# aleksandrina-streltsova/lidar-global-registration

Hardware: AMD Instinct MI355X
Metric: scan-pair registrations/sec (higher is better)
Workload: dtype f32

## Files before the change

lidar-global-registration_amd/csrc/lgr_match.hip:

```cpp
#include <rocprim/device/device_radix_sort.hpp>
#include <rocprim/device/device_scan.hpp>

#include <algorithm>
#include <vector>

#include "lgr_internal.h"

#include "lgr_match_common.cuh"
#include "lgr_match_cluster.cuh"
#include "lgr_match_pack.cuh"
#include "lgr_match_mfma.cuh"
#include "lgr_match_sweep.cuh"
#include "lgr_match_bounds.cuh"
#include "lgr_match_rerank.cuh"

extern "C" int lgr_match_last_stats(lgr_ctx* ctx, unsigned* out6) {
    if (!ctx || !out6) return LGR_ERR_INVALID_ARG;
    const lgr_match_stats& s = ctx->mstats;
    out6[0] = s.items_ab; out6[1] = s.dense_ab; out6[2] = s.items_ba;
    out6[3] = s.dense_ba; out6[4] = (unsigned) s.sub_cols; out6[5] = (unsigned) s.rg_rows;
    return LGR_OK;
}
extern "C" int lgr_match_last_work(lgr_ctx* ctx, double* executed_fraction) {
    if (!ctx || !executed_fraction) return LGR_ERR_INVALID_ARG;
// ... 347 lines not shown
    MaskStats* scratch_stats() const { return (MaskStats*) lb_part; }
};

struct CheckView {
    const uint8_t *done = nullptr, *sched = nullptr;
    const float* lb = nullptr;
    const unsigned* ustage = nullptr;
    const float *uq_rows = nullptr, *uq_cols = nullptr;
};

static const float betas[] = {LGR_PRUNE_BETAS};
static const int n_beta = (int) (sizeof betas / sizeof betas[0]);
static_assert(sizeof betas / sizeof betas[0] == 1, "LGR_PRUNE_BETAS: one final pass only (lgr_match_common.cuh)");
static_assert(sizeof betas / sizeof betas[0] + 1 <= 7, "MaskStats: slot 7 holds the stages counted once");

struct MatchCall {
    lgr_ctx* const ctx;
    const float* const d_a; const int ma;
    const float* const d_b; const int mb;
    const int block;
    int32_t* const d_ab_idx; float* const d_ab_dist; int32_t* const d_ba_idx; float* const d_ba_dist;
    const bool both;
    const lgr_match_options& mo;
    lgr_match_stats& st;
    const int near_t;
    const bool prune;
    MatchPrep* const P;
    const Side& A;
    Side B;
    int sub = 1, n_leaves = 0, rg_rows = BLOCK_ROWS;
    float *cen = nullptr, *cen2 = nullptr;
    char* misc = nullptr;
    int ma_pad = 0, mb_pad = 0, ta = 0, tb = 0, n_rb = 0, n_stage_total = 0, n_cc = 0, n_rg = 0, n_groups = 0, n_cpad = 0;
    float *sortedA = nullptr, *sortedB = nullptr;
    bool boxes = false;
    float *boxA = nullptr, *boxBt = nullptr;
    unsigned* rmax2 = nullptr;
    Fork aux;
    bool f16 = false, force_dense = false;
    OperandScale os{};
    int KS = 0, NF = 0;
    size_t bset_stride = 0, cset_stride = 0;
    char *Aop = nullptr, *Bop = nullptr;
    float *nAp = nullptr, *nBp = nullptr;
    float2 *shellA = nullptr, *shellB = nullptr;
    unsigned* d_max = nullptr;
    float *gmaxB = nullptr, *gmaxA = nullptr;
    int *cl_of_rg = nullptr, *tile_group = nullptr, *tile_leaf = nullptr, *group_start = nullptr;
    int *group_leaf = nullptr, *leaf_g0 = nullptr;
    Fork sB;
    PruneWs W{};
    int *rowmin = nullptr, *colmin = nullptr;
    unsigned long long *bestA = nullptr, *bestB = nullptr;
    int item_rb = 0, n_ir = 0, ccx = 0, n_flags = 0, mfma_grid = 0;
    int *iflags = nullptr, *ipos = nullptr;
    int2* ilist = nullptr;
    int *xcd_start = nullptr, *xcd_ctr = nullptr;
    unsigned kept_cap = 0;
    uint2* kept = nullptr;
    unsigned long long* kept_count = nullptr;
    unsigned short* ucol16 = nullptr;
    bool split_used = false;
    bool colstage = false, coarse = false;
    CoarseArgs ca_on{};
    ShellArgs shell{}, shell0{};
    const uint8_t* sched_final = nullptr;
    const unsigned long long* cur_pass_stages = nullptr;
    bool defer_init = false;
    CompView comp_rows{nullptr, 0, nullptr}, comp_cols{nullptr, 0, nullptr};
    CheckView chk;

    MatchCall(lgr_ctx* ctx, const float* d_a, int ma, const float* d_b, int mb, int block, int32_t* d_ab_idx, float* d_ab_dist, int32_t* d_ba_idx, float* d_ba_dist)
        : ctx(ctx), d_a(d_a), ma(ma), d_b(d_b), mb(mb), block(block), d_ab_idx(d_ab_idx), d_ab_dist(d_ab_dist), d_ba_idx(d_ba_idx), d_ba_dist(d_ba_dist),
          both(d_ba_idx != nullptr && mb > 0), mo(ctx->mopt), st(ctx->mstats), near_t(mo.near > 0 ? mo.near : NEAR_T),
          prune(mo.prune == 1 || (mo.prune != 0 && (double) ma * mb >= 65536.0 * 65536.0)),
          P(match_prep_of(ctx)), A(P->A) {}

    int build_both(const IrrRef* irr);
    int build_sides();
    int start_aux();
    int launch_sorted_copies(bool behind_main);
    int join_sorted();
    int choose_format();
    int upload_group_tables();
    PruneWs carve_prune_ws(char* base) const;
    int prepare_prune_ws();
    int pack_operands();
    int alloc_tables();
    int launch_mfma(const unsigned* mask, const CoarseArgs& ca, bool allow_split = true);
    int init_touched_tables();
    int run_dense();
    int lower_bounds();
    int coarse_setup();
    int near_schedule();
    CoarseArgs with_bounds() const;
    void build_comp();
    int upper_bounds_schedule(int pass);
    int init_pass_tables(int pass);
    int build_masks(int pass);
    int run_pruned();
    int read_back_stats();
    int irregular_rows();
    int self_check(const CheckView& v);
    int rerank();
};

#include "lgr_match_debug.cuh"

int MatchCall::build_both(const IrrRef* irr) {
    return lgr_run_pair(ctx, [&](lgr_ctx* cx) { return build_side(cx, d_a, ma, P->cen, P->cen2, P->sub, 1, P->rg_rows, WS_MATCH_NA, WS_MATCH_AP, 0, irr, &P->A); },
                        [&](lgr_ctx* cx) { return build_side(cx, d_b, mb, P->cen, P->cen2, P->sub, TILE, PAD, WS_MATCH_NB, WS_MATCH_BP, 1, irr, &B); });
}
int MatchCall::build_sides() {
    const bool prepared = P->armed && P->d_a == d_a && P->ma == ma && P->mb == mb && P->both == both && memcmp(&P->mopt, &mo, sizeof mo) == 0;
    P->armed = false;
    if (!prepared) LGR_TRY(match_cluster(ctx, d_a, ma, d_b, mb, both, true, P));
    LGR_TRY(build_both(P->irr));
    if (A.n_irr > IRR_CAP || B.n_irr > IRR_CAP || ((A.n_irr || B.n_irr) && (A.n_valid == 0 || B.n_valid == 0))) {
        st.irr_gave_up = 1u;
        LGR_TRY(build_both(nullptr));
    }
    st.irr_a = (unsigned) A.n_irr; st.irr_b = (unsigned) B.n_irr;
    sub = P->sub; n_leaves = KCL * sub; rg_rows = P->rg_rows;
    cen = P->cen; cen2 = P->cen2;
    LGR_TRY(lgr_ws_t(ctx, WS_MATCH_MISC, 8192, &misc));
    if (A.n_valid == 0 || B.n_valid == 0) return LGR_OK;
    ma_pad = A.n_pad; mb_pad = B.n_pad;
    st.rg_rows = rg_rows;
    ta = ma_pad / TILE; tb = mb_pad / TILE;
    n_rb = ma_pad / BLOCK_ROWS; n_stage_total = mb_pad / STAGE_COLS;
    return LGR_OK;
}

int MatchCall::start_aux() {
    LGR_TRY(lgr_ws_t(ctx, WS_MATCH_SORTED_B, (size_t) mb_pad * 33, &sortedB));
    if (both || prune) LGR_TRY(lgr_ws_t(ctx, WS_MATCH_SORTED_A, (size_t) ma_pad * 33, &sortedA));
    boxes = prune && mo.box_bounds != 0;
    if (boxes) {
        LGR_TRY(lgr_ws_t(ctx, WS_MATCH_BOX, (size_t) n_rb * 66 + (size_t) n_leaves * 66 + 64, &boxA));
        boxBt = boxA + (size_t) n_rb * 66;
        rmax2 = (unsigned*) (boxBt + (size_t) n_leaves * 66);
    }
    LGR_TRY(lgr_ctx_aux(ctx));
    aux.start(ctx, ctx->aux->stream, ctx->aux_ev, true);
    LGR_TRY(aux.fork(ctx->aux_ev));
    if (boxes) {
        const float* basis = P->basis;
        LGR_HIP(ctx, hipMemsetAsync(rmax2, 0, 4, aux.s));
        box_kernel<<<n_rb, 256, 0, aux.s>>>(d_a, A.perm, nullptr, n_rb, basis, basis + 33 * 33, 0, boxA, rmax2);
        box_kernel<<<n_leaves, 256, 0, aux.s>>>(d_b, B.perm, B.leaf_start, n_leaves, basis, basis + 33 * 33, 1, boxBt, rmax2);
        LGR_HIP(ctx, hipEventRecord(ctx->ev[30], aux.s));
    }
    LGR_HIP(ctx, hipGetLastError());
    return LGR_OK;
}
int MatchCall::launch_sorted_copies(bool behind_main) {
    if (aux.recorded) return LGR_OK;
    if (behind_main) LGR_TRY(aux.fork(ctx->ev[26]));
    gather_rows_kernel<<<cdiv((long long) mb_pad * 33, 256), 256, 0, aux.s>>>(d_b, B.perm, mb_pad, sortedB);
    if (sortedA) gather_rows_kernel<<<cdiv((long long) ma_pad * 33, 256), 256, 0, aux.s>>>(d_a, A.perm, ma_pad, sortedA);
    LGR_HIP(ctx, hipGetLastError());
    return aux.record();
}
int MatchCall::join_sorted() {
    LGR_TRY(launch_sorted_copies(false));
    return aux.join();
}

int MatchCall::choose_format() {
    f16 = mo.operand_format != 0;
    LGR_TRY(lgr_ws_t(ctx, WS_MATCH_NORMS, (size_t) ma_pad + (size_t) KCL * mb_pad + 2 * ((size_t) ta + (size_t) KCL * tb) + 64, &nAp));
    nBp = nAp + ma_pad;
    shellA = (float2*) (nBp + (size_t) KCL * mb_pad);
    shellB = shellA + ta;
    d_max = (unsigned*) (misc + 128);
    LGR_HIP(ctx, hipMemsetAsync(d_max, 0, 12, ctx->stream));
    const float r2 = std::max(A.nstat_n2, B.nstat_n2), drop2 = std::max(A.nstat_drop, B.nstat_drop);
    if (f16) force_dense = A.nstat_ovf || B.nstat_ovf;
    os = operand_scale(f16, r2, drop2, mo.operand_format);
    if (f16 && env_int("LGR_MATCH_DEBUG", 0))
        fprintf(stderr, "[lgr] operand statistics: max |x - c|^2 %.6g, dropped energy %.6g (A %.6g, B %.6g) -> %s; irregular rows %d + %d\n", (double) r2, (double) drop2,
                (double) A.nstat_drop, (double) B.nstat_drop, os.rot ? "rotated" : "plain", A.n_irr, B.n_irr);
    st.f16 = f16 ? (os.rot ? 2 : 1) : 0;
    KS = !f16 ? OpFmt<FMT_F32>::KS : os.rot ? OpFmt<FMT_F16R>::KS : OpFmt<FMT_F16>::KS;
    NF = !f16 ? OpFmt<FMT_F32>::NF : os.rot ? OpFmt<FMT_F16R>::NF : OpFmt<FMT_F16>::NF;
    const size_t frag_bytes = f16 ? sizeof(f16x8) : sizeof(float);
    const size_t a_op_bytes = (size_t) ta * NF * 64 * frag_bytes;
    bset_stride = (size_t) tb * NF * 64;
    LGR_TRY(lgr_ws_t(ctx, WS_MATCH_ROWMIN, a_op_bytes + 256, &Aop));
    const size_t b_op_bytes = KCL * bset_stride * frag_bytes;
    LGR_TRY(lgr_ws_t(ctx, WS_MATCH_COLMIN, b_op_bytes + 256, &Bop));
    n_rg = cdiv(ma_pad, rg_rows);
    return LGR_OK;
}

int MatchCall::upload_group_tables() {
    std::vector<int> h_group_start, h_tiles(2 * (size_t) tb);
    int group_cols = GROUP_COLS;
    while (group_cols < 65536 && ((size_t) mb_pad / group_cols + n_leaves) * (size_t) ma_pad * 4 > ((size_t) 24 << 30)) group_cols *= 2;
    for (int l = 0; l < n_leaves; ++l)
        for (int s0 = B.h_leaf_start[l]; s0 < B.h_leaf_start[l + 1]; s0 += group_cols) {
            int s1 = std::min(B.h_leaf_start[l + 1], s0 + group_cols), g = (int) h_group_start.size();
            h_group_start.push_back(s0);
            for (int t = s0 / TILE; t < s1 / TILE; ++t) { h_tiles[t] = g; h_tiles[tb + t] = l; }
        }
    n_groups = (int) h_group_start.size();
    st.sub_cols = n_groups;
    h_group_start.push_back(mb_pad);
    LGR_TRY(lgr_ws_t(ctx, WS_MATCH_BEST_B, (size_t) KCL * n_groups + 2 * (size_t) n_rg + 2 * (size_t) tb + 2 * (size_t) n_groups + n_leaves + 72, &gmaxB));
    gmaxA = gmaxB + (size_t) KCL * n_groups;
    cl_of_rg = (int*) (gmaxA + n_rg);
    tile_group = cl_of_rg + n_rg;
    tile_leaf = tile_group + tb;
    group_start = tile_leaf + tb;
    group_leaf = group_start + n_groups + 1;
    leaf_g0 = group_leaf + n_groups;
    std::vector<int> h(n_rg), hgl(n_groups), hl(n_leaves + 1, n_groups);
    for (int g = 0; g < n_rg; ++g) h[g] = A.h_blkcl[(size_t) g * (rg_rows / BLOCK_ROWS)];
    for (int g = 0; g < n_groups; ++g) hgl[g] = h_tiles[tb + h_group_start[g] / TILE];
    for (int g = n_groups - 1; g >= 0; --g) hl[hgl[g]] = g;
    for (int l = n_leaves - 1; l >= 0; --l) hl[l] = std::min(hl[l], hl[l + 1]);
    LGR_HIP(ctx, hipMemcpyAsync(cl_of_rg, h.data(), h.size() * 4, hipMemcpyHostToDevice, ctx->stream));
    LGR_HIP(ctx, hipMemcpyAsync(tile_group, h_tiles.data(), h_tiles.size() * 4, hipMemcpyHostToDevice, ctx->stream));
    LGR_HIP(ctx, hipMemcpyAsync(group_start, h_group_start.data(), h_group_start.size() * 4, hipMemcpyHostToDevice, ctx->stream));
    LGR_HIP(ctx, hipMemcpyAsync(group_leaf, hgl.data(), hgl.size() * 4, hipMemcpyHostToDevice, ctx->stream));
    LGR_HIP(ctx, hipMemcpyAsync(leaf_g0, hl.data(), hl.size() * 4, hipMemcpyHostToDevice, ctx->stream));
    LGR_HIP(ctx, hipStreamSynchronize(ctx->stream));
    return LGR_OK;
}

static void launch_pack16(bool rot, hipStream_t s, const float* X, const int* perm, int n_pad, int role, const float* cen, const int* blkcl, const F16Scale& sc,
                          void* op, float* nrm, float2* shell) {
    if (rot) pack16_kernel<true><<<cdiv(n_pad, 256), 256, 0, s>>>(X, perm, n_pad, role, cen, blkcl, sc, (_Float16*) op, nrm, shell);
    else pack16_kernel<false><<<cdiv(n_pad, 256), 256, 0, s>>>(X, perm, n_pad, role, cen, blkcl, sc, (_Float16*) op, nrm, shell);
}

PruneWs MatchCall::carve_prune_ws(char* base) const {
    Carve carve{0, base};
    PruneWs w{};
    const size_t n_pairs = (size_t) n_rb * n_leaves;
    w.LBsq = carve.take<float>(n_pairs * 4);
    w.done = carve.take<uint8_t>(n_pairs);
    w.sched = carve.take<uint8_t>(n_pairs);
    w.touched = carve.take<uint8_t>(n_pairs);
    w.mask = carve.take<unsigned>((size_t) n_rb * n_cc * 4);
    w.mask_acc = carve.take<unsigned>((size_t) n_rb * n_cc * 4);
    w.u_rb = carve.take<float>((size_t) n_rb * 4);
    w.u_rt = carve.take<float>((size_t) n_rb * (BLOCK_ROWS / TILE) * 4);
    w.u_leaf = carve.take<unsigned>((size_t) MAXLEAF * 4);
    w.stats = carve.take<MaskStats>(sizeof(MaskStats));
    w.lb_part = carve.take<uint2>((size_t) n_rb * sizeof(uint2));
    w.leaf_first = carve.take<int>((size_t) MAXLEAF * 4);
    w.leaf_last = carve.take<int>((size_t) MAXLEAF * 4);
    w.mask_chk = carve.take<unsigned>(mo.self_check ? (size_t) 2 * n_rb * n_cc * 4 + 256 : 0);
    w.u_stage = carve.take<unsigned>((size_t) n_stage_total * 4);
    w.u_ct = carve.take<unsigned>((size_t) tb * 4);
    w.comp_r = carve.take<uint8_t>((size_t) n_rb * n_groups);
    w.comp_c = carve.take<uint8_t>((size_t) n_leaves * n_rg);
    w.smaxB = carve.take<float>((size_t) KCL * n_stage_total * 4);
    w.coarse_cnt = carve.take<unsigned long long>(32);
    w.u_row = carve.take<float>((size_t) ma_pad * 4);
    w.u_colv = carve.take<float>((size_t) mb_pad * 4);
    w.stage_shell = carve.take<float2>((size_t) KCL * n_stage_total * 8);
    w.rb_shell = carve.take<float2>((size_t) n_rb * 8);
    w.cperm = carve.take<int>((size_t) (n_leaves + TILE) * 4);
    w.cnrm = carve.take<float>((size_t) KCL * (n_leaves + TILE) * 4);
    w.cop = carve.take<f16x8>((size_t) KCL * ((n_leaves + TILE) / TILE) * 7 * 64 * sizeof(f16x8));
    w.clear_begin = (char*) w.done; w.clear_end = (char*) w.comp_r;
    w.bytes = carve.off;
    return w;
}
int MatchCall::prepare_prune_ws() {
    hipStream_t s3 = ctx->stream;
    if (f16) LGR_TRY(lgr_ctx_stream3(ctx, &s3));
    sB.start(ctx, s3, ctx->ev3, s3 != ctx->stream);
    n_cc = cdiv(mb_pad, CHUNK_COLS);
    n_cpad = pad_to(n_leaves, TILE);
    cset_stride = (size_t) (n_cpad / TILE) * NF * 64;
    if (!prune) return LGR_OK;
    char* pb;
    LGR_TRY(lgr_ws_t(ctx, WS_MATCH_PRUNE, carve_prune_ws(nullptr).bytes, &pb));
    W = carve_prune_ws(pb);
    LGR_TRY(sB.fork(ctx->ev[31]));
    LGR_HIP(ctx, hipMemsetAsync(W.clear_begin, 0, W.clear_end - W.clear_begin, sB.s));
    if (f16) {
        centre_perm_kernel<<<cdiv(n_cpad, 256), 256, 0, sB.s>>>(n_leaves, n_cpad, W.cperm);
        launch_pack16(os.rot, sB.s, cen2, W.cperm, n_cpad, 1, cen, nullptr, os.sc, W.cop, W.cnrm, nullptr);
    }
    if (sB.live) LGR_HIP(ctx, hipEventRecord(ctx->ev[27], sB.s));
    return LGR_OK;
}

int MatchCall::pack_operands() {
    if (!f16) {
        pack_kernel<<<cdiv(ma_pad, 256), 256, 0, ctx->stream>>>(d_a, A.perm, ma_pad, 0, cen, A.blkcl, (float*) Aop, nAp, d_max + 2);
        pack_kernel<<<dim3(cdiv(mb_pad, 256), KCL), 256, 0, ctx->stream>>>(d_b, B.perm, mb_pad, 1, cen, nullptr, (float*) Bop, nBp, d_max + 2);
        unsigned* h_ovf;
        LGR_TRY(lgr_pinned(ctx, 64, (void**) &h_ovf));
        LGR_HIP(ctx, hipMemcpyAsync(h_ovf, d_max + 2, 4, hipMemcpyDeviceToHost, ctx->stream));
        LGR_HIP(ctx, hipStreamSynchronize(ctx->stream));
        force_dense = h_ovf[0] != 0u;
    } else {
        launch_pack16(os.rot, ctx->stream, d_a, A.perm, ma_pad, 0, cen, A.blkcl, os.sc, Aop, nAp, shellA);
        LGR_TRY(sB.fork(ctx->ev3));
        launch_pack16(os.rot, sB.s, d_b, B.perm, mb_pad, 1, cen, nullptr, os.sc, Bop, nBp, shellB);
    }
    group_max_kernel<<<dim3(n_groups, KCL), 256, 0, sB.s>>>(nBp, mb_pad, 0, group_start, gmaxB);
    group_max_kernel<<<dim3(n_rg, 1), 256, 0, ctx->stream>>>(nAp, ma_pad, rg_rows, nullptr, gmaxA);
    return LGR_OK;
}

int MatchCall::alloc_tables() {
    const size_t tab_floats = (size_t) n_groups * ma_pad + (both ? (size_t) n_rg * mb_pad : 0);
    LGR_TRY(lgr_ws_t(ctx, WS_MATCH_BEST_A, tab_floats + 2 * ((size_t) ma + mb) + 64, &rowmin));
    if (both) colmin = rowmin + (size_t) n_groups * ma_pad;
    bestA = (unsigned long long*) (rowmin + tab_floats + (tab_floats & 1));
    bestB = bestA + ma;
    fill_u64<<<cdiv(ma + mb, 256), 256, 0, sB.s>>>(bestA, ma + mb, ~0ull);
    if (!prune) LGR_HIP(ctx, hipMemsetD32Async((hipDeviceptr_t) rowmin, 0x7f800000, tab_floats, ctx->stream));
    else if (mo.poison_tables) LGR_HIP(ctx, hipMemsetD32Async((hipDeviceptr_t) rowmin, 0, tab_floats, ctx->stream));
    item_rb = both ? std::min(rg_rows / BLOCK_ROWS, 16) : 4;
    n_ir = cdiv(n_rb, item_rb); ccx = cdiv(n_cc, 8); n_flags = 8 * ccx * n_ir;
    int* ibuf;
    LGR_TRY(lgr_ws_t(ctx, WS_MATCH_ITEMS2, (size_t) 4 * n_flags + 128, &ibuf));
    iflags = ibuf; ipos = ibuf + n_flags;
    ilist = (int2*) (ibuf + 2 * (size_t) n_flags);
    xcd_start = ibuf + 4 * (size_t) n_flags;
    xcd_ctr = xcd_start + 16;
    mfma_grid = 8 * (LGR_MM_OCC / 2) * std::max(1, ctx->n_cu / 8);
    kept_cap = mo.kept_cap > 0 ? (unsigned) mo.kept_cap : (16u << 20);
    if (f16 && os.rot && prune && mo.coarse_rejection != 0 && mo.split_sweep != 0) {
        char* kb;
        LGR_TRY(lgr_ws_t(ctx, WS_MATCH_KEPT, (size_t) kept_cap * sizeof(uint2) + (size_t) mb_pad * 2 + 512, &kb));
        kept = (uint2*) kb;
        kept_count = (unsigned long long*) (kb + (size_t) kept_cap * sizeof(uint2));
        ucol16 = (unsigned short*) (kb + (size_t) kept_cap * sizeof(uint2) + 256);
    }
    st.stages_all = (double) n_rb * n_stage_total;
    return LGR_OK;
}

template <bool BOTH, int FMT, bool CO>
static void launch_match_mfma_as(const MatchCall& c, const unsigned* mask, const int* xs, const CoarseArgs& ca) {
    typedef typename OpFmt<FMT>::frag frag;
    match_mfma<BOTH, FMT, CO><<<c.mfma_grid, NTHR, 0, c.ctx->stream>>>((const frag*) c.Aop, (const frag*) c.Bop, c.bset_stride, c.os.c_scale, c.os.out_scale, c.A.blkcl, c.nAp,
                                                                       c.ma_pad, c.mb_pad, c.rg_rows, c.tile_group, mask, c.rowmin, c.colmin, c.n_cc, c.item_rb, c.ilist, xs, c.xcd_ctr, ca);
}
template <int FMT, bool CO>
static void launch_match_mfma_fmt(const MatchCall& c, const unsigned* mask, const int* xs, const CoarseArgs& ca) {
    if (c.both) launch_match_mfma_as<true, FMT, CO>(c, mask, xs, ca);
    else launch_match_mfma_as<false, FMT, CO>(c, mask, xs, ca);
}
static void launch_match_mfma(const MatchCall& c, bool co, const unsigned* mask, const int* xs, const CoarseArgs& ca) {
    if (!c.f16) launch_match_mfma_fmt<FMT_F32, false>(c, mask, xs, ca);
    else if (!c.os.rot) launch_match_mfma_fmt<FMT_F16, false>(c, mask, xs, ca);
    else if (co) launch_match_mfma_fmt<FMT_F16R, true>(c, mask, xs, ca);
    else launch_match_mfma_fmt<FMT_F16R, false>(c, mask, xs, ca);
}

int MatchCall::init_touched_tables() {
    LGR_HIP(ctx, hipMemsetAsync(W.touched, 0, (size_t) n_rb * n_leaves, ctx->stream));
    touched_kernel<<<4 * std::max(1, ctx->n_cu), 256, 0, ctx->stream>>>(kept, kept_count, kept_cap, xcd_start + 48, W.sched, tile_leaf, n_leaves, (size_t) n_rb * n_leaves, W.touched);
    init_tables_sparse_kernel<<<cdiv((long long) n_rb * n_leaves, 256), 256, 0, ctx->stream>>>(W.touched, W.done, n_rb, n_leaves, leaf_g0, group_start, rg_rows / BLOCK_ROWS, rowmin,
                                                                                               (size_t) ma_pad, colmin, (size_t) mb_pad);
    return LGR_OK;
}

int MatchCall::launch_mfma(const unsigned* mask, const CoarseArgs& ca, bool allow_split) {
    items_flag_kernel<<<cdiv(n_flags, 256), 256, 0, ctx->stream>>>(mask, n_rb, n_cc, item_rb, n_ir, ccx, iflags);
    size_t sb = 0;
    LGR_HIP(ctx, rocprim::exclusive_scan(nullptr, sb, iflags, ipos, 0, (size_t) n_flags, rocprim::plus<int>(), ctx->stream));
    void* stmp;
    LGR_TRY(lgr_ws(ctx, WS_GRID_TMP, sb, &stmp));
    LGR_HIP(ctx, rocprim::exclusive_scan(stmp, sb, iflags, ipos, 0, (size_t) n_flags, rocprim::plus<int>(), ctx->stream));
    items_emit_kernel<<<cdiv(n_flags, 256), 256, 0, ctx->stream>>>(iflags, ipos, item_rb, n_ir, ccx, ilist, xcd_start);
    LGR_HIP(ctx, hipMemsetAsync(xcd_ctr, 0, 32, ctx->stream));
    LGR_CHECK(ctx, ctx->mfma_timed < 8, LGR_ERR_INVALID_ARG);
    LGR_TRY(sB.join());
    (void) hipEventRecord(ctx->ev[9 + 2 * ctx->mfma_timed], ctx->stream);
    if (f16 && os.rot && ca.u_rb && kept && allow_split) {
        split_used = true;
        LGR_HIP(ctx, hipMemsetAsync(kept_count, 0, 8, ctx->stream));
        if (ca.u_colv) ucol_pack_kernel<<<cdiv(mb_pad, 256), 256, 0, ctx->stream>>>(ca.u_colv, mb_pad, os.c_scale, ucol16);
        int* xs_sweep = xcd_start + 32;
        int* xs_plain = xcd_start + 48;
        pass_select_kernel<<<1, 16, 0, ctx->stream>>>(mo.coarse_rejection == 2 ? nullptr : cur_pass_stages, 0.5 * st.stages_all, xcd_start, xs_sweep, xs_plain);
        const int sweep_grid = 8 * (SW_OCC / 2) * std::max(1, ctx->n_cu / 8);
        match_sweep<<<sweep_grid, NTHR, 0, ctx->stream>>>((const f16x8*) Aop, (const f16x8*) Bop, bset_stride, os.c_scale, A.blkcl, ma_pad, mb_pad, rg_rows, mask, n_cc,
                                                          item_rb, ilist, xs_sweep, xcd_ctr, ca, ca.u_colv ? ucol16 : nullptr, kept, kept_count, kept_cap);
        if (defer_init) LGR_TRY(init_touched_tables());
        const int tiles_grid = 8 * std::max(1, ctx->n_cu);
        if (both) match_tiles<true><<<tiles_grid, 64 * TL_WAVES, 0, ctx->stream>>>((const f16x8*) Aop, (const f16x8*) Bop, bset_stride, os.out_scale, A.blkcl, ma_pad, mb_pad,
                                                                                   rg_rows, tile_group, rowmin, colmin, kept, kept_count, kept_cap);
        else match_tiles<false><<<tiles_grid, 64 * TL_WAVES, 0, ctx->stream>>>((const f16x8*) Aop, (const f16x8*) Bop, bset_stride, os.out_scale, A.blkcl, ma_pad, mb_pad,
                                                                               rg_rows, tile_group, rowmin, colmin, kept, kept_count, kept_cap);
        launch_match_mfma(*this, false, mask, xs_plain, CoarseArgs{});
    } else {
        launch_match_mfma(*this, ca.u_rb != nullptr, mask, xcd_start, ca);
    }
    (void) hipEventRecord(ctx->ev[10 + 2 * ctx->mfma_timed], ctx->stream);
    ctx->mfma_timed += 1;
    LGR_HIP(ctx, hipGetLastError());
#ifdef EXP_PROF
    LGR_TRY(match_prof_report(ctx, xcd_start));
#endif
    return LGR_OK;
}

int MatchCall::run_dense() {
    LGR_TRY(launch_sorted_copies(true));
    LGR_TRY(launch_mfma(nullptr, CoarseArgs{}));
    st.stages_done = st.stages_unique = st.stages_all;
    return LGR_OK;
}

int MatchCall::lower_bounds() {
    if (sB.live) LGR_HIP(ctx, hipStreamWaitEvent(ctx->stream, ctx->ev[27], 0));
    if (!f16) {
        LGR_TRY(join_sorted());
        lb_kernel<<<n_rb, 256, 0, ctx->stream>>>(sortedA, A.perm, cen2, B.r2max, B.leaf_count, n_leaves, W.LBsq);
    } else if (os.rot) {
        lb_mfma_kernel<FMT_F16R><<<n_rb, LBM_THREADS, 0, ctx->stream>>>((const f16x8*) Aop, W.cop, cset_stride, os.out_scale, A.blkcl, nAp, W.cnrm, os.ex,
                                                                        B.r2max, B.leaf_count, n_leaves, n_cpad, W.LBsq);
    } else {
        lb_mfma_kernel<FMT_F16><<<n_rb, LBM_THREADS, 0, ctx->stream>>>((const f16x8*) Aop, W.cop, cset_stride, os.out_scale, A.blkcl, nAp, W.cnrm, os.ex,
                                                                       B.r2max, B.leaf_count, n_leaves, n_cpad, W.LBsq);
    }
    LGR_HIP(ctx, hipGetLastError());
    return LGR_OK;
}
int MatchCall::coarse_setup() {
    colstage = both && mo.column_stage != 0;
    coarse = f16 && os.rot && mo.coarse_rejection != 0;
    if (coarse) {
        shell_reduce_kernel<<<cdiv((long long) KCL * n_stage_total, 256), 256, 0, sB.s>>>(shellB, KCL, tb, STAGE_TILES, W.stage_shell, W.smaxB);
        LGR_HIP(ctx, hipMemsetAsync(W.coarse_cnt, 0, 32, ctx->stream));
        ca_on = coarse_constants(os);
        ca_on.xmax = gmaxA; ca_on.ymax = W.smaxB; ca_on.n_stage_total = n_stage_total;
        ca_on.cnt = W.coarse_cnt;
    }
    if (coarse && mo.shell_bound != 0) {
        shell_reduce_kernel<<<cdiv(n_rb, 256), 256, 0, ctx->stream>>>(shellA, 1, ta, BLOCK_ROWS / TILE, W.rb_shell, nullptr);
        shell.rshA = W.rb_shell; shell.sshB = W.stage_shell;
        shell.blkcl = A.blkcl; shell.u_rb = W.u_rb; shell.cols = both ? 1 : 0;
        ca_on.rt_shell = shellA; ca_on.ct_shell = shellB;
    }
    shell0 = shell;
    shell0.u_rb = nullptr;
    sched_final = W.sched;
    comp_rows = CompView{W.comp_r, n_groups, nullptr};
    comp_cols = CompView{W.comp_c, n_rg, tile_leaf};
    return LGR_OK;
}
CoarseArgs MatchCall::with_bounds() const {
    CoarseArgs ca = ca_on;
    ca.u_rb = W.u_rb; ca.u_rt = W.u_rt; ca.u_row = W.u_row; ca.u_stage = both ? W.u_stage : nullptr; ca.u_ct = W.u_ct; ca.u_colv = both ? W.u_colv : nullptr; ca.n_ct_total = tb;
    return ca;
}
static int launch_near(const MatchCall& c, int n_vec, int len, size_t vs, size_t es, unsigned long long* lbstat, const uint2* lb_part) {
// ... 104 lines not shown
    if (split_used) LGR_HIP(ctx, hipMemcpyAsync(h_kept, kept_count, 8, hipMemcpyDeviceToHost, ctx->stream));
    LGR_HIP(ctx, hipStreamSynchronize(ctx->stream));
    if (split_used && h_kept[0] > (unsigned long long) kept_cap) {
        LGR_HIP(ctx, hipMemsetAsync(W.coarse_cnt, 0, 32, ctx->stream));
        LGR_TRY(launch_mfma(W.mask, with_bounds(), false));
        LGR_HIP(ctx, hipMemcpyAsync(h_cc, W.coarse_cnt, 24, hipMemcpyDeviceToHost, ctx->stream));
        LGR_HIP(ctx, hipStreamSynchronize(ctx->stream));
    }
    st.coarse_tested = (double) h_cc[0];
    st.coarse_rejected = (double) h_cc[1];
    st.shell_skipped = (double) h_cc[2];
    st.stages_done = 0;
    for (int k = 0; k <= n_beta; ++k) st.stages_done += (double) hs->stages[k];
    st.stages_unique = (double) hs->stages[7];
    st.lb_zero = (double) hs->stages[5]; st.lb_finite = (double) hs->stages[6];
    if (env_int("LGR_MATCH_DEBUG", 0)) LGR_TRY(match_debug_report(*this, hs, h_kept));
    return LGR_OK;
}

int MatchCall::irregular_rows() {
    const int nb_a = (ma + block - 1) / block, nb_b = (mb + block - 1) / block;
    if (B.n_irr) irregular_scan<<<cdiv(ma, 256), 256, 0, ctx->stream>>>(d_a, A.valid, ma, d_b, B.irr_list, B.n_irr, block, nb_a, nb_b, bestA, both ? bestB : nullptr);
    if (A.n_irr) irregular_scan<<<cdiv(mb, 256), 256, 0, ctx->stream>>>(d_b, B.valid, mb, d_a, A.irr_list, A.n_irr, block, nb_b, nb_a, both ? bestB : nullptr, bestA);
    return LGR_OK;
}
int MatchCall::self_check(const CheckView& v) {
    unsigned* d_worst = (unsigned*) (misc + 192);
    unsigned long long* d_cover = (unsigned long long*) (misc + 3840);
    static_assert(2 * CHECK_N == 8, "lgr_match_last_check_cover reports four counters per direction");
    LGR_HIP(ctx, hipMemsetAsync(d_worst, 0, 8, ctx->stream));
    LGR_HIP(ctx, hipMemsetAsync(d_cover, 0, 2 * CHECK_N * 8, ctx->stream));
    const int stride = mo.self_check >= 2 ? 1 : 37;
    check_kernel<true><<<cdiv(ma_pad, stride), 256, (size_t) (n_groups + 8) * 4, ctx->stream>>>(
        (const float*) rowmin, n_groups, ma_pad, 0, group_start, sortedA, A.perm, sortedB, B.perm, mb_pad, nAp, A.blkcl, nullptr, gmaxB, nullptr,
        os.ex, comp_rows, stride, nullptr, nullptr, 0, nullptr, nullptr, v.uq_rows, v.uq_cols, d_worst, d_cover);
    if (both)
        check_kernel<false><<<cdiv(mb_pad, stride), 256, (size_t) (n_rg + 8) * 4, ctx->stream>>>(
            (const float*) colmin, n_rg, mb_pad, rg_rows, nullptr, sortedB, B.perm, sortedA, A.perm, ma_pad, nullptr, nullptr, nBp, gmaxA, cl_of_rg,
            os.ex, comp_cols, stride, v.done, v.sched, n_leaves, v.lb, v.ustage, v.uq_rows, v.uq_cols, d_worst + 1, d_cover + CHECK_N);
    unsigned* hw;
    LGR_TRY(lgr_pinned(ctx, 128, (void**) &hw));
    LGR_HIP(ctx, hipMemcpyAsync(hw, d_worst, 8, hipMemcpyDeviceToHost, ctx->stream));
    LGR_HIP(ctx, hipMemcpyAsync(hw + 16, d_cover, 2 * CHECK_N * 8, hipMemcpyDeviceToHost, ctx->stream));
    LGR_HIP(ctx, hipStreamSynchronize(ctx->stream));
    float r0, r1;
    memcpy(&r0, hw, 4); memcpy(&r1, hw + 1, 4);
    ctx->mcheck[0] = r0; ctx->mcheck[1] = r1;
    memcpy(ctx->mcover, hw + 16, (both ? 2 : 1) * CHECK_N * 8);
    return LGR_OK;
}
int MatchCall::rerank() {
    RefilterArgs ra{(const f16x8*) Aop, (const f16x8*) Bop, bset_stride, os.out_scale, (f16 && mo.rerank_refilter) ? KS : 0, A.blkcl, mo.pair_cap};
    auto rerank_ab = [&](lgr_ctx* cx) {
        return run_rerank<true>(cx, os.ex, comp_rows, (const float*) rowmin, n_groups, 0, group_start, d_a, A, nAp, nullptr, gmaxB, nullptr, d_b, sortedB, B, block, bestA,
                                d_ab_idx, d_ab_dist, &st.items_ab, &st.dense_ab, force_dense, ra, &st.pairs_ab);
    };
    auto rerank_ba = [&](lgr_ctx* cx) {
        return run_rerank<false>(cx, os.ex, comp_cols, (const float*) colmin, n_rg, rg_rows, nullptr, d_b, B, nullptr, nBp, gmaxA, cl_of_rg, d_a, sortedA, A, block, bestB,
                                 d_ba_idx, d_ba_dist, &st.items_ba, &st.dense_ba, force_dense, ra, &st.pairs_ba);
    };
    if (both) return lgr_run_pair(ctx, rerank_ab, rerank_ba);
    return rerank_ab(ctx);
}

static int match_impl(lgr_ctx* ctx, const float* d_a, int ma, const float* d_b, int mb, int block,
                      int32_t* d_ab_idx, float* d_ab_dist, int32_t* d_ba_idx, float* d_ba_dist) {
    LGR_CHECK(ctx, ctx && (d_a || ma == 0) && (d_b || mb == 0) && (d_ab_idx || ma == 0) && (d_ab_dist || ma == 0), LGR_ERR_INVALID_ARG);
    LGR_CHECK(ctx, ma >= 0 && mb >= 0 && block > 0, LGR_ERR_INVALID_ARG);
    if (d_ba_idx) LGR_CHECK(ctx, d_ba_dist != nullptr, LGR_ERR_INVALID_ARG);
    LGR_HIP(ctx, hipSetDevice(ctx->device));
    memset(&ctx->mstats, 0, sizeof ctx->mstats);
    ctx->mcheck[0] = ctx->mcheck[1] = -1;
    for (unsigned long long& c : ctx->mcover) c = ~0ull;
    ctx->mfma_timed = 0;
    if (ma) { LGR_HIP(ctx, hipMemsetAsync(d_ab_idx, 0xff, (size_t) ma * 4, ctx->stream)); LGR_HIP(ctx, hipMemsetAsync(d_ab_dist, 0, (size_t) ma * 4, ctx->stream)); }
    if (mb && d_ba_idx) { LGR_HIP(ctx, hipMemsetAsync(d_ba_idx, 0xff, (size_t) mb * 4, ctx->stream)); LGR_HIP(ctx, hipMemsetAsync(d_ba_dist, 0, (size_t) mb * 4, ctx->stream)); }
    if (ma == 0 || mb == 0) return LGR_OK;

    MatchCall c(ctx, d_a, ma, d_b, mb, block, d_ab_idx, d_ab_dist, d_ba_idx, d_ba_dist);
    LGR_TRY(c.build_sides());
    if (c.A.n_valid == 0 || c.B.n_valid == 0) return LGR_OK;
    LGR_TRY(c.start_aux());
    LGR_TRY(c.choose_format());
    LGR_TRY(c.upload_group_tables());
    LGR_TRY(c.prepare_prune_ws());
    LGR_TRY(c.pack_operands());
    LGR_TRY(c.alloc_tables());
    LGR_TRY(c.prune ? c.run_pruned() : c.run_dense());
    LGR_HIP(ctx, hipGetLastError());
    LGR_TRY(c.join_sorted());
    LGR_TRY(c.irregular_rows());
    if (c.mo.self_check && c.sortedA) LGR_TRY(c.self_check(c.chk));
    return c.rerank();
}

extern "C" int lgr_match_last_kernel_ms(lgr_ctx* ctx, float* ms) {
    if (!ctx || !ms) return LGR_ERR_INVALID_ARG;
    *ms = -1.f;
    if (!ctx->mfma_timed) return LGR_OK;
    *ms = 0.f;
    for (int k = 0; k < ctx->mfma_timed; ++k) {
        float t = 0.f;
        LGR_HIP(ctx, hipEventSynchronize(ctx->ev[10 + 2 * k]));
        LGR_HIP(ctx, hipEventElapsedTime(&t, ctx->ev[9 + 2 * k], ctx->ev[10 + 2 * k]));
        if (env_int("LGR_MATCH_DEBUG", 0)) fprintf(stderr, "[lgr] match_mfma pass %d: %.2f ms\n", k, t);
        *ms += t;
    }
    return LGR_OK;
}

extern "C" int lgr_match_bf_dev(lgr_ctx* ctx, const float* d_q33, int mq, const float* d_t33, int mt, int block,
                                int32_t* d_idx, float* d_dist) {
    lgr_turn turn__(ctx);
    if (!ctx) return LGR_ERR_INVALID_ARG;
    return match_impl(ctx, d_q33, mq, d_t33, mt, block, d_idx, d_dist, nullptr, nullptr);
}

extern "C" int lgr_match_bf2_dev(lgr_ctx* ctx, const float* d_a33, int ma, const float* d_b33, int mb, int block,
                                 int32_t* d_ab_idx, float* d_ab_dist, int32_t* d_ba_idx, float* d_ba_dist) {
    lgr_turn turn__(ctx);
    if (!ctx) return LGR_ERR_INVALID_ARG;
    LGR_CHECK(ctx, (d_ba_idx && d_ba_dist) || mb == 0, LGR_ERR_INVALID_ARG);
    return match_impl(ctx, d_a33, ma, d_b33, mb, block, d_ab_idx, d_ab_dist, d_ba_idx, d_ba_dist);
}

extern "C" int lgr_match_bf(lgr_ctx* ctx, const float* q33, int mq, const float* t33, int mt, int block,
                            int32_t* idx, float* dist) {
    lgr_turn turn__(ctx);
    if (!ctx) return LGR_ERR_INVALID_ARG;
    LGR_CHECK(ctx, (q33 || mq == 0) && (t33 || mt == 0) && (idx || mq == 0) && (dist || mq == 0) && mq >= 0 && mt >= 0, LGR_ERR_INVALID_ARG);
    LGR_HIP(ctx, hipSetDevice(ctx->device));
    float *dq, *dt, *dd;
    int32_t* di;
    LGR_TRY(lgr_ws_t(ctx, WS_HOST_A, (size_t) mq * 33 + 1, &dq));
    LGR_TRY(lgr_ws_t(ctx, WS_HOST_B, (size_t) mt * 33 + 1, &dt));
    LGR_TRY(lgr_ws_t(ctx, WS_HOST_C, (size_t) mq + 1, &di));
    LGR_TRY(lgr_ws_t(ctx, WS_HOST_D, (size_t) mq + 1, &dd));
    if (mq) LGR_HIP(ctx, hipMemcpyAsync(dq, q33, (size_t) mq * 132, hipMemcpyHostToDevice, ctx->stream));
    if (mt) LGR_HIP(ctx, hipMemcpyAsync(dt, t33, (size_t) mt * 132, hipMemcpyHostToDevice, ctx->stream));
    LGR_TRY(lgr_match_bf_dev(ctx, dq, mq, dt, mt, block, di, dd));
    if (mq) {
        LGR_HIP(ctx, hipMemcpyAsync(idx, di, (size_t) mq * 4, hipMemcpyDeviceToHost, ctx->stream));
        LGR_HIP(ctx, hipMemcpyAsync(dist, dd, (size_t) mq * 4, hipMemcpyDeviceToHost, ctx->stream));
    }
    LGR_HIP(ctx, hipStreamSynchronize(ctx->stream));
    return LGR_OK;
}
```

lidar-global-registration_amd/csrc/lgr_match_cluster.cuh:

```cuda
#pragma once
#include "lgr_match_common.cuh"

namespace {

struct KmAcc { long long sum[33]; long long cnt; };
__device__ __forceinline__ double km_scale(unsigned kmax_bits) {
    return kmax_bits ? ldexp(1.0, 40 - ((int) (kmax_bits >> 23) - 127)) : 1.0;
}
constexpr int IRR_CAND = 16;
constexpr int IRR_CAP = 1024;
struct IrrRef { double s[3]; double tol; int enabled; int best; unsigned n_ok; unsigned agree[IRR_CAND]; };
__device__ __forceinline__ void block_sums(const float* v, double& s0, double& s1, double& s2) {
    s0 = 0.0; s1 = 0.0; s2 = 0.0;
#pragma unroll
    for (int k = 0; k < 11; ++k) { s0 += (double) v[k]; s1 += (double) v[11 + k]; s2 += (double) v[22 + k]; }
}
__device__ __forceinline__ bool sums_agree(double a0, double a1, double a2, double r0, double r1, double r2, double tol) {
    return fabs(a0 - r0) <= tol && fabs(a1 - r1) <= tol && fabs(a2 - r2) <= tol;
}
__device__ __forceinline__ double sums_tol(double r0, double r1, double r2) { return 1e-5 * fmax(fmax(fabs(r0), fabs(r1)), fabs(r2)); }
__device__ __forceinline__ const float* sample_row(int s, const float* __restrict__ A, int ma, const float* __restrict__ B, int mb, int per_side) {
    const bool fromA = !B || s < per_side;
    const float* X = fromA ? A : B;
    const int m = fromA ? ma : mb;
// ... 243 lines not shown
        const int cc = threadIdx.x / 3, j = threadIdx.x % 3;
        double t = 0.0;
        for (int k = 0; k < 11; ++k) t += (double) cen[cc * 33 + 11 * j + k];
        cs_s[cc][j] = t;
    }
    __syncthreads();
    int i = blockIdx.x * blockDim.x + threadIdx.x;
    float st_n2 = 0.f, st_drop = 0.f;
    bool st_ovf = false;
    if (i < m) {
        float v[33], r2;
        bool ok = row_finite(X + (size_t) i * 33, v);
        unsigned key = 0xffffffffu;
        bool irr = false;
        double bx0 = 0.0, bx1 = 0.0, bx2 = 0.0;
        if (ok) block_sums(v, bx0, bx1, bx2);
        if (ok && irr_ref && irr_ref->enabled) {
            irr = !sums_agree(bx0, bx1, bx2, irr_ref->s[0], irr_ref->s[1], irr_ref->s[2], irr_ref->tol);
            if (irr) {
                const unsigned pos = atomicAdd(&nstat[3], 1u);
                if (pos < (unsigned) IRR_CAP) irr_list[pos] = i;
            }
        }
        if (ok && !irr) {
            int c = 0;
            r2 = __uint_as_float(0x7f800000u);
            float own_drop = 0.f;
#pragma unroll 1
            for (int cc = 0; cc < KCL; ++cc) {
                float d = 0.f;
#pragma unroll
                for (int k = 0; k < 33; ++k) {
                    const float t = v[k] - cen[cc * 33 + k];
                    d = d + t * t;
                }
                const double mg = 6.6e-7 * (double) sqrtf(d);
                const double s0 = fabs(bx0 - cs_s[cc][0]) + mg, s1 = fabs(bx1 - cs_s[cc][1]) + mg, s2 = fabs(bx2 - cs_s[cc][2]) + mg;
                const float dr = (float) (((s0 * s0 + s1 * s1) + s2 * s2) * (1.0001 / 11.0)) * 1.000001f + 1e-20f * d;
                if (d < r2) { r2 = d; c = cc; own_drop = dr; }
                if (role == 1) {
                    if (d < FLT_BIG) st_n2 = fmaxf(st_n2, d); else st_ovf = true;
                    st_drop = fmaxf(st_drop, dr);
                }
            }
            if (role == 0) {
                if (r2 < FLT_BIG) st_n2 = r2; else st_ovf = true;
                st_drop = own_drop;
            }
            float rl2;
            int j = nearest_sub(v, c2s + c * pitch, sub, rl2);
            if (!(r2 < FLT_BIG)) r2 = __uint_as_float(0x7f800000u);
            if (!(rl2 < FLT_BIG)) rl2 = __uint_as_float(0x7f800000u);
            int leaf = c * sub + j;
            key = ((unsigned) leaf << 22) | (__float_as_uint(r2) >> 9);
            atomicAdd(&lc[leaf], 1);
            atomicMax(&lr[leaf], __float_as_uint(rl2));
        }
        if (!ok || irr) atomicAdd(&lc[MAXLEAF], 1);
        keys[i] = key; vals[i] = i; valid[i] = ok ? (irr ? 2 : 1) : 0;
    }
    __syncthreads();
    for (int l = threadIdx.x; l <= MAXLEAF; l += blockDim.x) {
        if (lc[l]) atomicAdd(&counts[l], lc[l]);
        if (l < MAXLEAF && lr[l]) atomicMax(&rmax[l], lr[l]);
    }
    for (int o = 32; o > 0; o >>= 1) { st_n2 = fmaxf(st_n2, __shfl_xor(st_n2, o)); st_drop = fmaxf(st_drop, __shfl_xor(st_drop, o)); }
    const bool any_ovf = __ballot(st_ovf) != 0ull;
    if ((threadIdx.x & 63) == 0) {
        if (st_n2 > 0.f && __float_as_uint(st_n2) > *(volatile unsigned*) &nstat[0]) atomicMax(&nstat[0], __float_as_uint(st_n2));
        if (st_drop > 0.f && __float_as_uint(st_drop) > *(volatile unsigned*) &nstat[1]) atomicMax(&nstat[1], __float_as_uint(st_drop));
        if (any_ovf) nstat[2] = 1u;
    }
}

__global__ void place_kernel(const unsigned* __restrict__ keys_sorted, const int* __restrict__ vals_sorted, int n_valid,
                             const int* __restrict__ sorted_start , const int* __restrict__ pad_start ,
                             int* __restrict__ perm) {
    int s = blockIdx.x * blockDim.x + threadIdx.x;
    if (s >= n_valid) return;
    int l = (int) (keys_sorted[s] >> 22);
    perm[pad_start[l] + (s - sorted_start[l])] = vals_sorted[s];
}


}
```

lidar-global-registration_amd/csrc/lgr_match_mfma.cuh:

```cuda
#pragma once
#include "lgr_match_common.cuh"

namespace {

#ifdef EXP_PROF
__device__ unsigned long long g_prof[16];
#define PROF_T(var) unsigned long long var = wall_clock64()
#define PROF_ADD(slot, a, b) do { if (tid == 0) atomicAdd(&g_prof[slot], (b) - (a)); } while (0)
#define PROF_CNT(slot) do { if (tid == 0) atomicAdd(&g_prof[slot], 1ull); } while (0)
#else
#define PROF_T(var)
#define PROF_ADD(slot, a, b)
#define PROF_CNT(slot)
#endif
__device__ __forceinline__ f32x16 mfma_step(float a, float b, f32x16 c) { return __builtin_amdgcn_mfma_f32_32x32x2f32(a, b, c, 0, 0, 0); }
__device__ __forceinline__ f32x16 mfma_step(f16x8 a, f16x8 b, f32x16 c) { return __builtin_amdgcn_mfma_f32_32x32x16_f16(a, b, c, 0, 0, 0); }
template <int FMT>
__device__ __forceinline__ f32x16 mfma_chain(const typename OpFmt<FMT>::frag (&a)[OpFmt<FMT>::NF], const typename OpFmt<FMT>::frag (&b)[OpFmt<FMT>::NF], f32x16 acc) {
#pragma unroll
    for (int kk = 0; kk < OpFmt<FMT>::KS; ++kk) acc = mfma_step(a[OpFmt<FMT>::fa(kk)], b[OpFmt<FMT>::fb(kk)], acc);
    return acc;
}

template <bool COLDIR, int FMT, bool CO >
// ... 357 lines not shown
                PROF_T(t_k0);
                unsigned any = kept[0] | kept[1] | kept[2] | kept[3];
                int prev_grp = -1;
                while (any) {
                    const int ks_ = __builtin_ctz(any);
                    any &= any - 1u;
#pragma unroll
                    for (int ct = 0; ct < STAGE_TILES; ++ct) {
                        if (!((kept[ct] >> ks_) & 1u)) continue;
                        const int grp = __builtin_amdgcn_readfirstlane(tg_s[ks_ * STAGE_TILES + ct]);
                        if (grp != prev_grp && prev_grp >= 0) flush_rows(prev_grp);
                        prev_grp = grp;
                        const frag* bsrc = Bset + (size_t) ks_ * STAGE_FRAGS + (size_t) ct * NF * 64 + lane;
                        frag b[NF];
#pragma unroll
                        for (int kk = 0; kk < NF; ++kk) b[kk] = bsrc[kk * 64];
                        const f32x16 acc = mfma_chain<FMT>(a, b, nav);
                        row_min1(acc);
                        col_min(acc, ks_, ct);
                    }
                }
                if (prev_grp >= 0) flush_rows(prev_grp);
                PROF_T(t_k1);
                PROF_ADD(5, t_k0, t_k1);
            }
            PROF_T(t_v2);
            PROF_ADD(1, t_v1, t_v2);
        }
    }
    if (COLDIR && col_dirty) {
        PROF_T(t_c0);
        asm volatile("s_waitcnt lgkmcnt(0)" : : : "memory");
        __syncthreads();
        int rg = rb0 / rg_blocks;
        int ncols = n_coltiles * TILE;
        int* dst = colmin + (size_t) rg * mb_pad + col_tile0 * TILE;
        constexpr int NCM = CHUNK_COLS / NTHR;
#pragma unroll
        for (int j = 0; j < NCM; ++j) {
            int i = tid + NTHR * j;
            const int cur = i < ncols ? cmin_s[i] : IINF;
            if (cur != IINF) {
                const int v = F16 ? __float_as_int(__int_as_float(cur) * out_scale) : cur;
                atomicMin(&dst[i], v);
                cmin_s[i] = IINF;
            }
        }
        PROF_T(t_c1);
        PROF_ADD(3, t_c0, t_c1);
    }
  }
    if (use_coarse && ca.cnt && lane == 0) {
        if (n_tested) atomicAdd(&ca.cnt[0], (unsigned long long) n_tested);
        if (n_rejected) atomicAdd(&ca.cnt[1], (unsigned long long) n_rejected);
        if (n_skipped) atomicAdd(&ca.cnt[2], (unsigned long long) n_skipped);
    }
    PROF_T(t_wg1);
    PROF_ADD(4, t_wg0, t_wg1);
}

__global__ void items_flag_kernel(const unsigned* __restrict__ mask, int n_rb, int n_cc, int item_rb, int n_ir, int ccx, int* __restrict__ flags) {
    int j = blockIdx.x * blockDim.x + threadIdx.x;
    if (j >= 8 * ccx * n_ir) return;
    int xcd = j / (ccx * n_ir), rem = j % (ccx * n_ir);
    int cc = (rem / n_ir) * 8 + xcd, ir = rem % n_ir;
    int f = 0;
    if (cc < n_cc) {
        if (!mask) f = 1;
        else
            for (int r = ir * item_rb; r < min(n_rb, (ir + 1) * item_rb); ++r) f |= mask[(size_t) r * n_cc + cc] != 0u ? 1 : 0;
    }
    flags[j] = f;
}
__global__ void items_emit_kernel(const int* __restrict__ flags, const int* __restrict__ pos, int item_rb, int n_ir, int ccx,
                                  int2* __restrict__ items, int* __restrict__ xcd_start ) {
    int j = blockIdx.x * blockDim.x + threadIdx.x;
    const int per_xcd = ccx * n_ir;
    if (j >= 8 * per_xcd) return;
    int xcd = j / per_xcd, rem = j % per_xcd;
    if (flags[j]) items[pos[j]] = make_int2((rem / n_ir) * 8 + xcd, (rem % n_ir) * item_rb);
    if (rem == 0) xcd_start[xcd] = pos[j];
    if (j == 8 * per_xcd - 1) xcd_start[8] = pos[j] + flags[j];
}


}
```

Baseline: 45.88.

## Build group tables on device and fuse item-list compaction into one kernel

Replaces the host-side construction and upload of group/tile/leaf tables, which ended in a stream synchronize, with a device kernel that computes the tables from leaf starts using a block prefix scan. The item list for the MFMA launch is now built by a single-block fused flag-plus-ballot-scan kernel when the flag count is small, replacing the flag kernel, the rocprim scan, the emit kernel and a memset. This removes a host stall and several launches per match call. In exchange it adds a serial single-block compaction that may be slow for larger flag counts, and it relies on every leaf start being a multiple of the tile size.

```diff
diff --git a/lidar-global-registration_amd/csrc/lgr_match.hip b/lidar-global-registration_amd/csrc/lgr_match.hip
--- a/lidar-global-registration_amd/csrc/lgr_match.hip
+++ b/lidar-global-registration_amd/csrc/lgr_match.hip
@@ -453,7 +453,7 @@
     int launch_sorted_copies(bool behind_main);
     int join_sorted();
     int choose_format();
-    int upload_group_tables();
+    int build_group_tables();
     PruneWs carve_prune_ws(char* base) const;
     int prepare_prune_ws();
     int pack_operands();
@@ -565,19 +565,12 @@
     return LGR_OK;
 }
 
-int MatchCall::upload_group_tables() {
-    std::vector<int> h_group_start, h_tiles(2 * (size_t) tb);
+int MatchCall::build_group_tables() {
     int group_cols = GROUP_COLS;
     while (group_cols < 65536 && ((size_t) mb_pad / group_cols + n_leaves) * (size_t) ma_pad * 4 > ((size_t) 24 << 30)) group_cols *= 2;
-    for (int l = 0; l < n_leaves; ++l)
-        for (int s0 = B.h_leaf_start[l]; s0 < B.h_leaf_start[l + 1]; s0 += group_cols) {
-            int s1 = std::min(B.h_leaf_start[l + 1], s0 + group_cols), g = (int) h_group_start.size();
-            h_group_start.push_back(s0);
-            for (int t = s0 / TILE; t < s1 / TILE; ++t) { h_tiles[t] = g; h_tiles[tb + t] = l; }
-        }
-    n_groups = (int) h_group_start.size();
+    n_groups = 0;
+    for (int l = 0; l < n_leaves; ++l) n_groups += groups_of_leaf(B.h_leaf_start[l], B.h_leaf_start[l + 1], group_cols);
     st.sub_cols = n_groups;
-    h_group_start.push_back(mb_pad);
     LGR_TRY(lgr_ws_t(ctx, WS_MATCH_BEST_B, (size_t) KCL * n_groups + 2 * (size_t) n_rg + 2 * (size_t) tb + 2 * (size_t) n_groups + n_leaves + 72, &gmaxB));
     gmaxA = gmaxB + (size_t) KCL * n_groups;
     cl_of_rg = (int*) (gmaxA + n_rg);
@@ -586,17 +579,9 @@
     group_start = tile_leaf + tb;
     group_leaf = group_start + n_groups + 1;
     leaf_g0 = group_leaf + n_groups;
-    std::vector<int> h(n_rg), hgl(n_groups), hl(n_leaves + 1, n_groups);
-    for (int g = 0; g < n_rg; ++g) h[g] = A.h_blkcl[(size_t) g * (rg_rows / BLOCK_ROWS)];
-    for (int g = 0; g < n_groups; ++g) hgl[g] = h_tiles[tb + h_group_start[g] / TILE];
-    for (int g = n_groups - 1; g >= 0; --g) hl[hgl[g]] = g;
-    for (int l = n_leaves - 1; l >= 0; --l) hl[l] = std::min(hl[l], hl[l + 1]);
-    LGR_HIP(ctx, hipMemcpyAsync(cl_of_rg, h.data(), h.size() * 4, hipMemcpyHostToDevice, ctx->stream));
-    LGR_HIP(ctx, hipMemcpyAsync(tile_group, h_tiles.data(), h_tiles.size() * 4, hipMemcpyHostToDevice, ctx->stream));
-    LGR_HIP(ctx, hipMemcpyAsync(group_start, h_group_start.data(), h_group_start.size() * 4, hipMemcpyHostToDevice, ctx->stream));
-    LGR_HIP(ctx, hipMemcpyAsync(group_leaf, hgl.data(), hgl.size() * 4, hipMemcpyHostToDevice, ctx->stream));
-    LGR_HIP(ctx, hipMemcpyAsync(leaf_g0, hl.data(), hl.size() * 4, hipMemcpyHostToDevice, ctx->stream));
-    LGR_HIP(ctx, hipStreamSynchronize(ctx->stream));
+    group_tables_kernel<<<std::min(cdiv(std::max(tb, n_rg), GT_THREADS), 32), GT_THREADS, 0, ctx->stream>>>(B.leaf_start, n_leaves, group_cols, tb, A.blkcl, n_rg, rg_rows / BLOCK_ROWS,
+                                                                                                    tile_group, tile_leaf, group_start, group_leaf, leaf_g0, cl_of_rg);
+    LGR_HIP(ctx, hipGetLastError());
     return LGR_OK;
 }
 
@@ -738,14 +723,18 @@
 }
 
 int MatchCall::launch_mfma(const unsigned* mask, const CoarseArgs& ca, bool allow_split) {
-    items_flag_kernel<<<cdiv(n_flags, 256), 256, 0, ctx->stream>>>(mask, n_rb, n_cc, item_rb, n_ir, ccx, iflags);
-    size_t sb = 0;
-    LGR_HIP(ctx, rocprim::exclusive_scan(nullptr, sb, iflags, ipos, 0, (size_t) n_flags, rocprim::plus<int>(), ctx->stream));
-    void* stmp;
-    LGR_TRY(lgr_ws(ctx, WS_GRID_TMP, sb, &stmp));
-    LGR_HIP(ctx, rocprim::exclusive_scan(stmp, sb, iflags, ipos, 0, (size_t) n_flags, rocprim::plus<int>(), ctx->stream));
-    items_emit_kernel<<<cdiv(n_flags, 256), 256, 0, ctx->stream>>>(iflags, ipos, item_rb, n_ir, ccx, ilist, xcd_start);
-    LGR_HIP(ctx, hipMemsetAsync(xcd_ctr, 0, 32, ctx->stream));
+    if (n_flags <= ITEMS_FUSED_MAX) {
+        items_fused_kernel<<<1, ITEMS_FUSED_THREADS, 0, ctx->stream>>>(mask, n_rb, n_cc, item_rb, n_ir, ccx, ilist, xcd_start, xcd_ctr);
+    } else {
+        items_flag_kernel<<<cdiv(n_flags, 256), 256, 0, ctx->stream>>>(mask, n_rb, n_cc, item_rb, n_ir, ccx, iflags);
+        size_t sb = 0;
+        LGR_HIP(ctx, rocprim::exclusive_scan(nullptr, sb, iflags, ipos, 0, (size_t) n_flags, rocprim::plus<int>(), ctx->stream));
+        void* stmp;
+        LGR_TRY(lgr_ws(ctx, WS_GRID_TMP, sb, &stmp));
+        LGR_HIP(ctx, rocprim::exclusive_scan(stmp, sb, iflags, ipos, 0, (size_t) n_flags, rocprim::plus<int>(), ctx->stream));
+        items_emit_kernel<<<cdiv(n_flags, 256), 256, 0, ctx->stream>>>(iflags, ipos, item_rb, n_ir, ccx, ilist, xcd_start);
+        LGR_HIP(ctx, hipMemsetAsync(xcd_ctr, 0, 32, ctx->stream));
+    }
     LGR_CHECK(ctx, ctx->mfma_timed < 8, LGR_ERR_INVALID_ARG);
     LGR_TRY(sB.join());
     (void) hipEventRecord(ctx->ev[9 + 2 * ctx->mfma_timed], ctx->stream);
@@ -1016,7 +1005,7 @@
     if (c.A.n_valid == 0 || c.B.n_valid == 0) return LGR_OK;
     LGR_TRY(c.start_aux());
     LGR_TRY(c.choose_format());
-    LGR_TRY(c.upload_group_tables());
+    LGR_TRY(c.build_group_tables());
     LGR_TRY(c.prepare_prune_ws());
     LGR_TRY(c.pack_operands());
     LGR_TRY(c.alloc_tables());
diff --git a/lidar-global-registration_amd/csrc/lgr_match_cluster.cuh b/lidar-global-registration_amd/csrc/lgr_match_cluster.cuh
--- a/lidar-global-registration_amd/csrc/lgr_match_cluster.cuh
+++ b/lidar-global-registration_amd/csrc/lgr_match_cluster.cuh
@@ -349,5 +349,47 @@
     perm[pad_start[l] + (s - sorted_start[l])] = vals_sorted[s];
 }
 
-
-}
+__host__ __device__ __forceinline__ int groups_of_leaf(int begin, int end, int group_cols) { return (end - begin + group_cols - 1) / group_cols; }
+constexpr int GT_THREADS = 1024;
+static_assert(MAXLEAF <= GT_THREADS, "group_tables_kernel: one thread per leaf");
+static_assert(GROUP_COLS % TILE == 0, "a column tile lies in one group");
+__global__ __launch_bounds__(GT_THREADS) void group_tables_kernel(const int* __restrict__ leaf_start , int n_leaves, int group_cols, int tb,
+                                                                  const int* __restrict__ blkcl, int n_rg, int blocks_per_rg,
+                                                                  int* __restrict__ tile_group, int* __restrict__ tile_leaf, int* __restrict__ group_start,
+                                                                  int* __restrict__ group_leaf, int* __restrict__ leaf_g0, int* __restrict__ cl_of_rg) {
+    __shared__ int ls[MAXLEAF + 1];
+    __shared__ int g0s[MAXLEAF + 1];
+    __shared__ int wave_sum[GT_THREADS / 64];
+    const int tid = threadIdx.x, lane = tid & 63, wave = tid >> 6;
+    for (int l = tid; l <= n_leaves; l += GT_THREADS) ls[l] = leaf_start[l];
+    __syncthreads();
+    const int ng = tid < n_leaves ? groups_of_leaf(ls[tid], ls[tid + 1], group_cols) : 0;
+    int incl = ng;
+    for (int o = 1; o < 64; o <<= 1) { const int t = __shfl_up(incl, o); if (lane >= o) incl += t; }
+    if (lane == 63) wave_sum[wave] = incl;
+    __syncthreads();
+    int g0 = incl - ng, n_groups = 0;
+    for (int w = 0; w < GT_THREADS / 64; ++w) { const int c = wave_sum[w]; if (w < wave) g0 += c; n_groups += c; }
+    if (tid < n_leaves) g0s[tid] = g0;
+    if (tid == 0) g0s[n_leaves] = n_groups;
+    __syncthreads();
+    if (blockIdx.x == 0) {
+        if (tid <= n_leaves) leaf_g0[tid] = g0s[tid];
+        if (tid < n_leaves)
+            for (int k = 0; k < ng; ++k) { group_start[g0 + k] = ls[tid] + k * group_cols; group_leaf[g0 + k] = tid; }
+        if (tid == 0) group_start[n_groups] = ls[n_leaves];
+    }
+    const int stride = gridDim.x * GT_THREADS;
+    for (int r = blockIdx.x * GT_THREADS + tid; r < n_rg; r += stride) cl_of_rg[r] = blkcl[(size_t) r * blocks_per_rg];
+    for (int t = blockIdx.x * GT_THREADS + tid; t < tb; t += stride) {
+        const int col = t * TILE;
+        int lo = 0, hi = n_leaves;
+        while (lo < hi) { const int mid = (lo + hi) >> 1; if (ls[mid] <= col) lo = mid + 1; else hi = mid; }
+        const int l = lo - 1;
+        tile_leaf[t] = l;
+        tile_group[t] = g0s[l] + (col - ls[l]) / group_cols;
+    }
+}
+
+
+}
diff --git a/lidar-global-registration_amd/csrc/lgr_match_mfma.cuh b/lidar-global-registration_amd/csrc/lgr_match_mfma.cuh
--- a/lidar-global-registration_amd/csrc/lgr_match_mfma.cuh
+++ b/lidar-global-registration_amd/csrc/lgr_match_mfma.cuh
@@ -463,6 +463,44 @@
     if (rem == 0) xcd_start[xcd] = pos[j];
     if (j == 8 * per_xcd - 1) xcd_start[8] = pos[j] + flags[j];
 }
-
-
+constexpr int ITEMS_FUSED_THREADS = 1024, ITEMS_FUSED_MAX = 16 * ITEMS_FUSED_THREADS;
+__global__ __launch_bounds__(ITEMS_FUSED_THREADS) void items_fused_kernel(const unsigned* __restrict__ mask, int n_rb, int n_cc, int item_rb, int n_ir, int ccx,
+                                                                          int2* __restrict__ items, int* __restrict__ xcd_start , int* __restrict__ xcd_ctr ) {
+    __shared__ int wave_sum[ITEMS_FUSED_THREADS / 64];
+    __shared__ int base_s;
+    const int tid = threadIdx.x, lane = tid & 63, wave = tid >> 6;
+    const int per_xcd = ccx * n_ir, n_flags = 8 * per_xcd;
+    if (tid < 8) xcd_ctr[tid] = 0;
+    if (tid == 0) base_s = 0;
+    __syncthreads();
+    for (int j0 = 0; j0 < n_flags; j0 += ITEMS_FUSED_THREADS) {
+        const int j = j0 + tid;
+        int f = 0, xcd = 0, rem = 0;
+        if (j < n_flags) {
+            xcd = j / per_xcd; rem = j % per_xcd;
+            const int cc = (rem / n_ir) * 8 + xcd, ir = rem % n_ir;
+            if (cc < n_cc) {
+                if (!mask) f = 1;
+                else
+                    for (int r = ir * item_rb; r < min(n_rb, (ir + 1) * item_rb); ++r) f |= mask[(size_t) r * n_cc + cc] != 0u ? 1 : 0;
+            }
+        }
+        const unsigned long long b = __ballot(f);
+        const int in_wave = __popcll(b & ((1ull << lane) - 1ull));
+        if (lane == 0) wave_sum[wave] = __popcll(b);
+        __syncthreads();
+        int pos = base_s + in_wave, total = 0;
+        for (int w = 0; w < ITEMS_FUSED_THREADS / 64; ++w) { const int c = wave_sum[w]; if (w < wave) pos += c; total += c; }
+        if (j < n_flags) {
+            if (f) items[pos] = make_int2((rem / n_ir) * 8 + xcd, (rem % n_ir) * item_rb);
+            if (rem == 0) xcd_start[xcd] = pos;
+            if (j == n_flags - 1) xcd_start[8] = pos + f;
+        }
+        __syncthreads();
+        if (tid == 0) base_s += total;
+        __syncthreads();
+    }
 }
+
+
+}
```

Result: no change. 45.77, median of 2 (-0.2%).
